# RViMLab/MICCAI2021_Cataract_semantic_segmentation

Measured on AMD Instinct MI355X. Metric: train frames/sec @540x960 OCRNet-HRNetw48, higher is better.
Workload: dtype f32 (convolutions with K >= 2048 and >= 192 output columns, and the 3x3 trunk convolutions of the HRNet widths: forward / backward-data of those with > 192 output columns: operands scaled by a per-tensor power of two and split into 2 fp16 planes (22 significant bits), 3 fp16 MFMA products; forward /

## Files before the change

include/catseg_debug.h:

```cpp
#ifndef CATSEG_DEBUG_H
#define CATSEG_DEBUG_H

#include "catseg.h"

#ifdef __cplusplus
extern "C" {
#endif

int catseg_debug_set_tile(int mi, int ni);
int catseg_debug_set_splits(int splits);
int catseg_debug_set_strided_multi(int on);
int catseg_debug_set_lovasz_prune(int on);
int catseg_debug_set_wgrad_direct(int on);

int catseg_debug_set_dconv3_blocks(int blocks);
int catseg_debug_set_dconv3_spec(int on);
int catseg_debug_set_dconv3_alt96(int on);
int catseg_debug_set_dwgrad3_blocks(int blocks);
int catseg_debug_set_dwgrad3_pl_blocks(int blocks);
int catseg_debug_set_dconv3_pl_slots(int slots);
int catseg_debug_set_dconv3_pl_pair(int mask);
int catseg_debug_dconv3_pl_occupancy(int C, int pair);
int catseg_debug_dwgrad3_pl_occupancy(int C);

int catseg_debug_set_h2w_slow_epilogue(int on);

int catseg_debug_set_b3_tile(int t);
int catseg_debug_plan_conv(const catseg_conv_desc* d, int op, int* out);

int catseg_debug_set_bilinear_bwd_fused(int on);
int catseg_debug_set_h2w_waves(int waves);

int catseg_debug_set_pconv1_wgrad_blocks(int n);

#ifdef __cplusplus
}
#endif
#endif
```

miccai2021_cataract_semantic_segmentation_amd/_lib.py:

```python
import ctypes as C
import os

import torch

_HERE = os.path.dirname(os.path.abspath(__file__))
LIB_PATH = os.environ.get("CATSEG_LIB") or os.path.join(_HERE, "libcatseg_hip.so")

if not os.path.exists(LIB_PATH):
    raise ImportError(
        "libcatseg_hip.so is missing (%s). Build it with `python -c 'import __graft_entry__ as g; g.build()'` "
        "or `make -C miccai2021_cataract_semantic_segmentation_amd/csrc`. There is no CPU fallback." % LIB_PATH)

lib = C.CDLL(LIB_PATH)

P, I, L, F, SZ = C.c_void_p, C.c_int, C.c_longlong, C.c_float, C.c_size_t


class ConvDesc(C.Structure):
    _fields_ = [(n, I) for n in ("B", "H", "W", "Cin", "Ho", "Wo", "Cout", "kh", "kw", "stride", "pad", "dil",
                                 "ldx", "ldy", "stem4", "groups")]


_SIGS = {
    "catseg_last_error": (C.c_char_p, []),
    "catseg_version": (I, []),
    "catseg_conv2d_fwd": (I, [P, P, P, P, P, I, P]),
    "catseg_conv2d_fwd_bnstats": (I, [P, P, P, P, P, I, P, SZ, P, P, P]),
    "catseg_conv2d_fwd_bf16x3_bnstats": (I, [P, P, P, P, P, I, P, SZ, P, P, P]),
    "catseg_bn_finalize": (I, [P, I, L, L, I, P, F, F, P, P, P, P, P]),
    "catseg_bn_finalize_counts": (I, [P, I, P, L, I, P, F, F, P, P, P, P, P]),
    "catseg_dconv3_supported": (I, [I]),
    "catseg_dconv3_wimg_bytes": (SZ, [I]),
    "catseg_dconv3_tiles": (I, [I, I, I, I, P, P]),
    "catseg_dconv3_prep": (I, [P, I, I, P, P]),
    "catseg_dconv3_layout": (I, [I, P, P]),
    "catseg_dwgrad3_supported": (I, [I]),
    "catseg_dwgrad3_workspace": (SZ, [I, I, I, I]),
    "catseg_dwgrad3": (I, [I, I, I, I, P, I, P, I, P, P, SZ, P]),
    "catseg_debug_set_dwgrad3_blocks": (I, [I]),
    "catseg_dconv3_prep_batch": (I, [P, I, P, P, P]),
    "catseg_dconv3": (I, [I, I, I, I, P, I, P, P, P, I, I, P, SZ, P, P]),
    "catseg_dconv3_bnbwd": (I, [I, I, I, I, P, I, P, P, I, P, I, P, P, P, P, SZ, P]),
    "catseg_dwgrad3_f16x2": (I, [I, I, I, I, P, I, P, P, I, P, P, P, SZ, P]),
    "catseg_dconv3_f16x2_wimg_bytes": (SZ, [I]),
    "catseg_dconv3_f16x2_prep_batch": (I, [P, I, P, P, P, P]),
    "catseg_dconv3_f16x2": (I, [I, I, I, I, P, I, P, P, P, P, P, I, I, P, SZ, P, P]),
    "catseg_dconv3_bnbwd_f16x2": (I, [I, I, I, I, P, I, P, P, P, P, I, P, I, P, P, P, P, SZ, P]),
    "catseg_dconv3_pl_supported": (I, [I]),
    "catseg_dconv3_pl_rows": (I, [I, I, I, I]),
    "catseg_planes_bytes": (SZ, [L, I]),
    "catseg_planes_from_f32": (I, [P, I, L, I, P, P, I, P]),
    "catseg_dconv3_pl": (I, [I, I, I, I, P, P, P, P, P, P, I, I, P, SZ, P, P, P]),
    "catseg_dconv3_pl_bnbwd": (I, [I, I, I, I, P, P, P, P, P, I, P, I, P, P, P, P, SZ, P, P]),
    "catseg_dwgrad3_pl_supported": (I, [I]),
    "catseg_dwgrad3_pl_workspace": (SZ, [I, I, I, I]),
    "catseg_dwgrad3_pl": (I, [I, I, I, I, P, P, P, P, P, P, SZ, P]),
    "catseg_bn_finalize_counts_bound": (I, [P, I, P, L, I, P, P, F, F, P, P, P, P, P, P, P]),
    "catseg_bn_apply_planes": (I, [P, I, P, P, P, P, I, P, P, I, P, L, I, I, P, P]),
    "catseg_add_n_act_planes": (I, [P, P, P, I, P, I, P, L, I, I, P, P]),
    "catseg_bn_backward_planes": (I, [P, I, P, I, P, I, P, P, P, L, I, I, P, P, P, P, P, P, P, I, I, P, SZ, P]),
    "catseg_bn_backward_pre_planes": (I, [P, I, P, I, P, P, P, I, L, I, P, P, P, P, P, P, P, SZ, P]),
    "catseg_bn_backward_h2_workspace": (SZ, [L, I]),
    "catseg_bn_backward_h2": (I, [P, I, P, I, P, I, P, P, P, L, I, I, P, P, P, P, P, P, P, P, P, SZ, P]),
    "catseg_head_fwd": (I, [P, I, P, P, P, P, P, I, L, I, P, I, I, P]),
    "catseg_head_backward_workspace": (SZ, [L, I]),
    "catseg_head_backward": (I, [P, I, P, I, P, P, P, P, I, L, I, P, P, P, P, P, P, P, P, P, P, P, SZ, P]),
    "catseg_head_fwd_drop": (I, [P, I, P, P, P, P, P, I, L, I, P, I, I, P, L, F, P]),
    "catseg_head_backward_drop": (I, [P, I, P, I, P, P, P, P, I, L, I, P, P, P, P, P, P, P, P, P, P, P, SZ, P, L, F, P]),
    "catseg_dropout2d_mask": (I, [P, F, I, I, P, P, P]),
    "catseg_dropout2d_mask_fixed": (I, [P, F, I, I, P, P, P]),
    "catseg_dropout2d_apply": (I, [P, I, P, L, I, L, P, I, P]),
    "catseg_maxpool2x2_fwd": (I, [P, I, P, I, P, I, I, I, I, P]),
    "catseg_maxpool2x2_bwd": (I, [P, I, P, P, I, I, I, I, I, P]),
    "catseg_bias_rows": (I, [P, P, I, L, I, P]),
    "catseg_bn_apply_amax": (I, [P, I, P, P, P, P, I, P, I, L, I, I, P, P]),
    "catseg_bn_backward_amax": (I, [P, I, P, I, P, I, P, P, P, L, I, I, P, I, P, P, P, I, I, P, SZ, P, P]),
    "catseg_bn_mask_bytes": (SZ, [L, I]),
    "catseg_bn_apply_mask": (I, [P, I, P, P, P, P, I, P, I, L, I, P, P, P]),
    "catseg_bn_backward_mask": (I, [P, I, P, P, I, P, P, L, I, P, I, P, P, P, I, I, P, SZ, P, P]),
    "catseg_bn_apply_planes_mask": (I, [P, I, P, P, P, P, I, P, P, I, P, L, I, P, P, P]),
    "catseg_bn_backward_planes_mask": (I, [P, I, P, P, I, P, P, L, I, P, P, P, P, P, P, P, I, I, P, SZ, P]),
    "catseg_bn_backward_pre_amax": (I, [P, I, P, I, P, P, P, I, L, I, P, I, P, P, P, SZ, P, P]),
    "catseg_add_n_act_amax": (I, [P, P, I, P, I, L, I, I, P, P]),
    "catseg_conv2d_fwd_fused": (I, [P, P, P, P, P, I, I, P, P]),
    "catseg_fold_bn": (I, [P, P, P, P, P, P, F, I, I, P, P, P]),
    "catseg_conv2d_bwd_data": (I, [P, P, P, P, I, P]),
    "catseg_conv2d_bwd_weight_workspace": (SZ, [P]),
    "catseg_conv2d_bwd_weight": (I, [P, P, P, P, P, P, SZ, P]),
    "catseg_gemm_batched": (I, [I, I, I, I, I, P, I, L, P, I, L, P, I, L, I, I, P]),
    "catseg_sum_slabs": (I, [P, P, L, I, I, I, P]),
    "catseg_debug_set_tile": (I, [I, I]),
    "catseg_debug_set_splits": (I, [I]),
    "catseg_debug_set_strided_multi": (I, [I]),
    "catseg_debug_set_lovasz_prune": (I, [I]),
    "catseg_debug_set_wgrad_direct": (I, [I]),
    "catseg_debug_plan_conv": (I, [P, I, P]),
    "catseg_debug_set_b3_tile": (I, [I]),
    "catseg_debug_set_dconv3_blocks": (I, [I]),
    "catseg_debug_set_dconv3_pl_slots": (I, [I]),
    "catseg_debug_set_dconv3_pl_pair": (I, [I]),
    "catseg_debug_set_dwgrad3_pl_blocks": (I, [I]),
    "catseg_debug_dconv3_pl_occupancy": (I, [I, I]),
    "catseg_debug_dwgrad3_pl_occupancy": (I, [I]),
    "catseg_debug_set_dconv3_spec": (I, [I]),
    "catseg_debug_set_dconv3_alt96": (I, [I]),
    "catseg_aug_pad_flip_u8": (I, [P, P, I, I, I, I, P, I, I, P]),
    "catseg_aug_box_blur": (I, [P, P, I, I, I, I, P, P, P, P]),
    "catseg_aug_color_op": (I, [P, I, I, I, P, P, P, SZ, P]),
    "catseg_split3_elems": (SZ, [L, I]),
    "catseg_split3": (I, [P, I, L, I, P, P]),
    "catseg_split3_weight_t": (I, [P, I, I, I, P, P]),
    "catseg_split3_blocked_elems": (SZ, [L, I]),
    "catseg_split3_blocked": (I, [P, L, I, I, P, P, P]),
    "catseg_split3_weight_blocked": (I, [P, I, I, I, P, P]),
    "catseg_split3_weight_t_blocked": (I, [P, I, I, I, P, P]),
    "catseg_conv2d_fwd_bf16x3_blocked": (I, [P, P, P, P, P, I, P, SZ, P, P, P]),
    "catseg_conv2d_bwd_data_bf16x3_blocked": (I, [P, P, P, P, I, P]),
    "catseg_conv2d_fwd_fused_bf16x3_blocked": (I, [P, P, P, P, P, I, I, P, P]),
    "catseg_split2h_blocked_elems": (SZ, [L, I]),
    "catseg_split2h_planar_elems": (SZ, [L, I]),
    "catseg_split2h": (I, [P, L, I, I, P, P, P, P]),
    "catseg_split2h_bound": (I, [P, L, I, I, P, P, P, P, P, P, P, P]),
    "catseg_conv2d_bwd_weight_f16x2_workspace": (SZ, [P]),
    "catseg_conv2d_bwd_weight_f16x2": (I, [P, P, P, P, P, P, P, SZ, P]),
    "catseg_conv2d_bwd_weight_f16x2_blocked": (I, [P, P, P, P, P, P, P, SZ, P]),
    "catseg_concat_bilinear_split2h": (I, [I, P, P, P, P, P, P, I, I, I, P, P, P]),
    "catseg_stem3_supported": (I, [I, I, I]),
    "catseg_stem3_partial_rows": (I, [I, I, I]),
    "catseg_stem3_wgrad_workspace": (SZ, []),
    "catseg_stem3_fwd": (I, [P, L, L, L, L, I, I, I, P, P, P, I, P, P, P]),
    "catseg_stem3_bwd_weight": (I, [P, L, L, L, L, I, I, I, P, I, P, P, SZ, P]),
    "catseg_stem7_supported": (I, [I, I, I]),
    "catseg_stem7_partial_rows": (I, [I, I, I]),
    "catseg_stem7_fwd": (I, [P, L, L, L, L, I, I, I, P, P, P, I, P, P, P]),
    "catseg_split2h_weight_blocked": (I, [P, I, I, I, P, P, P]),
    "catseg_split2h_weight_t_blocked": (I, [P, I, I, I, P, P, P]),
    "catseg_conv2d_fwd_f16x2_blocked": (I, [P, P, P, P, P, P, P, I, P, SZ, P, P, P]),
    "catseg_conv2d_fwd_fused_f16x2_blocked": (I, [P, P, P, P, P, P, P, I, I, P, P]),
    "catseg_conv2d_bwd_data_f16x2_blocked": (I, [P, P, P, P, P, P, I, P]),
    "catseg_conv2d_fwd_bf16x3": (I, [P, P, P, P, P, I, P]),
    "catseg_conv2d_bwd_data_bf16x3": (I, [P, P, P, P, I, P]),
    "catseg_conv2d_bwd_weight_bf16x3_workspace": (SZ, [P]),
    "catseg_conv2d_bwd_weight_bf16x3": (I, [P, P, P, P, P, SZ, P]),
    "catseg_bias_grad": (I, [P, I, L, I, P, P, SZ, P]),
    "catseg_bn_workspace": (SZ, [L, I]),
    "catseg_bn_train_stats": (I, [P, L, I, I, P, F, F, P, P, P, P, P, SZ, P]),
    "catseg_bn_eval_scale": (I, [I, P, P, F, P, P]),
    "catseg_bn_apply": (I, [P, I, P, P, P, P, I, P, I, L, I, I, P]),
    "catseg_bn_backward": (I, [P, I, P, I, P, I, P, P, P, L, I, I, P, I, P, P, P, I, I, P, SZ, P]),
    "catseg_bn_backward_pre": (I, [P, I, P, I, P, P, P, I, L, I, P, I, P, P, P, SZ, P]),
    "catseg_nchw3_to_nhwc4": (I, [P, P, I, I, I, P]),
    "catseg_nchw3_to_nhwc4_norm": (I, [P, P, I, I, I, P, P, P]),
    "catseg_stem_pack_weight": (I, [P, P, I, P]),
    "catseg_stem_unpack_grad": (I, [P, P, I, P]),
    "catseg_axpy2d": (I, [P, I, P, I, L, I, F, I, P]),
    "catseg_add_n_act": (I, [P, P, I, P, I, L, I, I, P]),
    "catseg_relu_bwd": (I, [P, I, P, I, P, I, L, I, P]),
    "catseg_weight_pad_cin": (I, [P, P, I, I, I, I, I, P]),
    "catseg_scale_by_device_scalar": (I, [P, L, P, P]),
    "catseg_maxpool3x3s2_fwd": (I, [P, I, P, I, P, I, I, I, I, I, I, P]),
    "catseg_maxpool3x3s2_bwd": (I, [P, I, P, P, I, I, I, I, I, I, I, P]),
    "catseg_bilinear_fwd": (I, [P, I, P, I, I, I, I, I, I, I, I, I, P]),
    "catseg_bilinear_bwd": (I, [P, I, P, I, I, I, I, I, I, I, I, I, I, P, SZ, P]),
    "catseg_global_avgpool_fwd": (I, [P, I, P, I, I, I, P]),
    "catseg_global_avgpool_bwd": (I, [P, P, I, I, I, I, I, P]),
    "catseg_adaptive_avgpool_fwd": (I, [P, I, P, I, I, I, I, I, P]),
    "catseg_adaptive_avgpool_bwd": (I, [P, P, I, I, I, I, I, I, I, P]),
    "catseg_softmax_spatial_workspace": (SZ, [I, I]),
    "catseg_softmax_spatial_fwd": (I, [P, P, I, I, I, I, P, SZ, P]),
    "catseg_softmax_spatial_bwd": (I, [P, P, P, I, I, I, I, I, P, SZ, P]),
    "catseg_softmax_rows_fwd": (I, [P, P, L, I, I, F, P]),
    "catseg_softmax_rows_bwd": (I, [P, P, P, L, I, I, F, P]),
    "catseg_lovasz_workspace": (SZ, [L, I]),
    "catseg_lovasz_softmax": (I, [P, P, L, I, F, P, P, I, P, SZ, P]),
    "catseg_lovasz_softmax_fwd": (I, [P, P, L, I, F, P, I, P, SZ, P]),
    "catseg_lovasz_softmax_bwd": (I, [P, L, I, F, P, P, I, P, SZ, P]),
    "catseg_ce_workspace": (SZ, [L]),
    "catseg_cross_entropy": (I, [P, P, L, I, L, F, P, P, P, SZ, P]),
    "catseg_ohem_workspace": (SZ, [L]),
    "catseg_ohem_cross_entropy": (I, [P, P, L, I, L, F, L, F, P, P, P, SZ, P]),
    "catseg_overlap_workspace": (SZ, [L, I]),
    "catseg_overlap_fwd": (I, [P, P, L, I, L, I, I, I, P, P, P, P, P, SZ, P]),
    "catseg_overlap_bwd": (I, [P, P, L, I, L, P, P, P, P]),
    "catseg_focal_workspace": (SZ, [L]),
    "catseg_focal_fwd": (I, [P, P, L, I, F, P, P, P, P, SZ, P]),
    "catseg_focal_bwd": (I, [P, P, L, I, F, P, P, P, P]),
    "catseg_ingest_u8": (I, [P, P, I, I, I, P, P, I, I, P, P, P, P, P, P]),
    "catseg_resize_nearest": (I, [P, I, P, I, I, I, I, I, I, I, I, I, F, P]),
    "catseg_ensemble_merge": (I, [P, P, I, L, I, I, P, I, P, P]),
    "catseg_confusion_matrix": (I, [P, P, L, I, P, P]),
    "catseg_adam_step": (I, [P, P, P, P, L, F, F, F, F, I, F, P]),
    "catseg_pconv1_supported": (I, [I, I]),
    "catseg_pconv1_wimg_bytes": (SZ, [I, I]),
    "catseg_pconv1_prep_batch": (I, [P, I, P, P, P, P]),
    "catseg_pconv1": (I, [L, I, I, P, I, P, P, P, P, P, I, I, P, SZ, P, P, P]),
    "catseg_pconv1_wgrad_supported": (I, [I, I]),
    "catseg_pconv1_wgrad_workspace": (SZ, [L, I, I]),
    "catseg_pconv1_wgrad": (I, [L, I, I, P, I, P, P, I, P, P, P, SZ, P]),
    "catseg_debug_set_pconv1_wgrad_blocks": (I, [I]),
    "catseg_debug_set_h2w_waves": (I, [I]),
    "catseg_debug_set_h2w_slow_epilogue": (I, [I]),
    "catseg_debug_set_bilinear_bwd_fused": (I, [I]),
    "catseg_gconv_supported": (I, [P]),
    "catseg_gconv_class_bytes": (SZ, [P]),
    "catseg_gconv_wimg_bytes": (SZ, [P, I]),
    "catseg_gconv_entries": (I, [P, I, L, L, P]),
    "catseg_gconv_fwd": (I, [P, P, P, P, P, P, P, P, SZ, P, P, P]),
    "catseg_gconv_bwd_data": (I, [P, P, P, P, P, P, I, P]),
    "catseg_gconv_wgrad_supported": (I, [P]),
    "catseg_gconv_wgrad_workspace": (SZ, [P]),
    "catseg_gconv_bwd_weight": (I, [P, P, P, P, P, P, P, SZ, P]),
    "catseg_adam_hyper": (None, [F, F, F, I, F, P]),
    "catseg_adam_step_dev": (I, [P, P, P, P, L, P, F, F, F, P]),
    "catseg_lds_limits": (I, [P, P]),
}
for _name, (_res, _args) in _SIGS.items():
    _fn = getattr(lib, _name)
    _fn.restype = _res
    _fn.argtypes = _args

EXPORTS = tuple(_SIGS)

if os.environ.get("CATSEG_SYNC"):
    class _SyncLib:
        def __init__(self, inner):
            self._inner = inner

        def __getattr__(self, name):
            fn = getattr(self._inner, name)
            if name in ("catseg_last_error", "catseg_version") or name.endswith("_workspace"):
                return fn

            def call(*a):
                desc = [[getattr(x._obj, f) for f, _ in x._obj._fields_] for x in a if isinstance(getattr(x, "_obj", None), ConvDesc)]
                print("[catseg]", name, desc, [x for x in a if isinstance(x, (int, float))], flush=True)
                rc = fn(*a)
                torch.cuda.synchronize()
                return rc
            return call

    lib = _SyncLib(lib)


class CatsegError(RuntimeError):
    pass


def check(rc):
    if rc != 0:
        raise CatsegError("libcatseg_hip: error %d: %s" % (rc, lib.catseg_last_error().decode()))


def stream():
    return torch.cuda.current_stream().cuda_stream


def ptr(t):
    return 0 if t is None else t.data_ptr()
```

miccai2021_cataract_semantic_segmentation_amd/csrc/dwgrad3_pl.hip:

```cpp
#include "planes.h"
#include "slabs.h"

extern int catseg_g_wg_blocks;
int catseg_g_wp96_blocks = 512;
extern "C" int catseg_debug_set_dwgrad3_pl_blocks(int blocks) {
  catseg_g_wp96_blocks = blocks > 0 ? blocks : 512;
  return CATSEG_OK;
}

namespace {

typedef _Float16 h8 __attribute__((ext_vector_type(8)));
typedef short s16x4 __attribute__((ext_vector_type(4)));
typedef short s16x8 __attribute__((ext_vector_type(8)));
typedef __attribute__((address_space(3))) s16x4 lds_s16x4;

constexpr int wp_rowbytes(int c) { return ((c * 2 / 32) & 1) ? c * 2 : c * 2 + 32; }

template <int COT_, int NCI_, int NTY_, int WM_, int WN_, int TH_, int NBUF_>
struct WpCfg {
  static constexpr int NBUF = NBUF_;
  static constexpr int COT = COT_, NCI = NCI_, NTY = NTY_, WM = WM_, WN = WN_, TH = TH_, TW = 16;
  static constexpr int NW = WM * WN, NTHR = 64 * NW;
  static_assert(NW == 4 && (TH == 2 || TH == 4), "four waves; tiles of 2 or 4 rows");
  static constexpr int MT = COT / 16 / WM;
  static constexpr int NTL = NTY * 3 * (NCI / 16);
  static constexpr int NTW = (NTL + WN - 1) / WN;
  static constexpr int XH = TH + NTY - 1, XW = TW + 2;
  static constexpr int NPX_X = XH * XW, NPX_D = TH * TW;
  static constexpr int ROWB_X = wp_rowbytes(NCI), ROWB_D = wp_rowbytes(COT);
  static constexpr int SX = ROWB_X / 16, SD = ROWB_D / 16;
  static constexpr int XPS = (NPX_X * ROWB_X + 255) / 256 * 256, DPS = (NPX_D * ROWB_D + 255) / 256 * 256;
  static constexpr int D0 = 2 * XPS, BUF = 2 * (XPS + DPS);
  static constexpr int LDS = NBUF * BUF;
  static constexpr int NKS = TH * TW / 32;
  static constexpr int NJX = (NPX_X * SX + 63) / 64, NJD = (NPX_D * SD + 63) / 64;
  static constexpr int MX = (NJX + 3) / 4, MD = (NJD + 3) / 4;
  static_assert(COT % (16 * WM) == 0 && NCI % 16 == 0 && (NTY == 1 || NTY == 3) && LDS <= 80 * 1024, "tiling");
};

struct WpArgs {
  const unsigned char* xp;
  const unsigned char* dp;
  unsigned P16;
  const int* x_rec;
  const int* d_rec;
  int B, H, W, C;
  int tiles_y, tiles_x, splits;
  float* slabs;
  long long slab_stride;
};

template <class G>
__global__ __launch_bounds__(G::NTHR, 2) void dwgrad3_pl_kernel(const WpArgs a) {
  __shared__ __attribute__((aligned(256))) unsigned char smem[G::LDS];
  const int tid = threadIdx.x, lane = tid & 63;
  const int wave = __builtin_amdgcn_readfirstlane(tid >> 6);
  const int wm = wave / G::WN, wn = wave % G::WN;
  const int i16 = lane & 15, kg = lane >> 4;

  const int nco = a.C / G::COT, nci = a.C / G::NCI;
  const int nvar = nco * nci * (G::NTY == 3 ? 1 : 3);
  const int split = (int)(blockIdx.x >> 3) / nvar * 8 + (int)(blockIdx.x & 7);
  if (split >= a.splits) return;
  int v = (int)(blockIdx.x >> 3) % nvar;
  const int cot0 = (v % nco) * G::COT; v /= nco;
  const int ci0 = (v % nci) * G::NCI; v /= nci;
  const int ky0 = G::NTY == 3 ? 0 : v;
  const int NG = a.C / 8;

  const int ntile = a.B * a.tiles_y * a.tiles_x;
  const int t_begin = (int)((long long)split * ntile / a.splits), t_end = (int)((long long)(split + 1) * ntile / a.splits);
  const int ex_x = __builtin_amdgcn_readfirstlane(a.x_rec[CS_REC_EXP]);
  const int ex_d = __builtin_amdgcn_readfirstlane(a.d_rec[CS_REC_EXP]);
  const bool one_step = ex_x + ex_d >= -120 && ex_x + ex_d <= 120;
  const float sc_out = __builtin_ldexpf(1.f, one_step ? -(ex_x + ex_d) : 0);

  int x_rel[G::MX], x_r[G::MX], x_c[G::MX], d_rel[G::MD], d_r[G::MD], d_c[G::MD];
  unsigned x_go[G::MX], d_go[G::MD];
#pragma unroll
  for (int m = 0; m < G::MX; ++m) {
    const int s = (wave + 4 * m) * 64 + lane, px = s / G::SX, g = s - px * G::SX;
    const bool live = px < G::NPX_X && g < G::NCI / 8;
    x_r[m] = live ? px / G::XW + ky0 - 1 : -(1 << 20);
    x_c[m] = px % G::XW - 1;
    x_rel[m] = ((px / G::XW + ky0 - 1) * a.W + (px % G::XW - 1)) * 16;
    x_go[m] = (unsigned)g * a.P16;
  }
#pragma unroll
  for (int m = 0; m < G::MD; ++m) {
    const int s = (wave + 4 * m) * 64 + lane, px = s / G::SD, g = s - px * G::SD;
    const bool live = px < G::NPX_D && g < G::COT / 8;
    d_r[m] = live ? px / G::TW : -(1 << 20);
    d_c[m] = px % G::TW;
    d_rel[m] = ((px / G::TW) * a.W + px % G::TW) * 16;
    d_go[m] = (unsigned)g * a.P16;
  }
  const unsigned plane_bytes = (unsigned)NG * a.P16;
  const __amdgpu_buffer_rsrc_t rsx = __builtin_amdgcn_make_buffer_rsrc((void*)a.xp, (short)0, (int)(2u * plane_bytes), 0x00020000);
  const __amdgpu_buffer_rsrc_t rsd = __builtin_amdgcn_make_buffer_rsrc((void*)a.dp, (short)0, (int)(2u * plane_bytes), 0x00020000);
  auto dma = [&](int tile, int buf) {
    const int tx = tile % a.tiles_x, ty = (tile / a.tiles_x) % a.tiles_y, b = tile / (a.tiles_x * a.tiles_y);
    const int y0 = ty * G::TH, x0 = tx * G::TW;
    const int org = (y0 * a.W + x0) * 16;
    const unsigned img = (unsigned)(b * a.H * a.W) * 16u;
    unsigned char* base = smem + buf * G::BUF;
#pragma unroll
    for (int m = 0; m < G::MX; ++m) {
      const int j = wave + 4 * m;
      if (j < G::NJX) {
        const bool ok = (unsigned)(y0 + x_r[m]) < (unsigned)a.H && (unsigned)(x0 + x_c[m]) < (unsigned)a.W;
        const unsigned voff = ok ? (unsigned)(org + x_rel[m]) + x_go[m] : 0xFFFFFFF0u;
#pragma unroll
        for (int p = 0; p < 2; ++p)
          if (j * 64 + lane < G::NPX_X * G::SX)
            __builtin_amdgcn_raw_ptr_buffer_load_lds(rsx, (__attribute__((address_space(3))) void*)(base + p * G::XPS + j * 1024), 16, voff,
                                                     (unsigned)(p * NG + ci0 / 8) * a.P16 + img, 0, 0);
      }
    }
#pragma unroll
    for (int m = 0; m < G::MD; ++m) {
      const int j = wave + 4 * m;
      if (j < G::NJD) {
        const bool ok = (unsigned)(y0 + d_r[m]) < (unsigned)a.H && (unsigned)(x0 + d_c[m]) < (unsigned)a.W;
        const unsigned voff = ok ? (unsigned)(org + d_rel[m]) + d_go[m] : 0xFFFFFFF0u;
#pragma unroll
        for (int p = 0; p < 2; ++p)
          if (j * 64 + lane < G::NPX_D * G::SD)
            __builtin_amdgcn_raw_ptr_buffer_load_lds(rsd, (__attribute__((address_space(3))) void*)(base + G::D0 + p * G::DPS + j * 1024), 16, voff,
                                                     (unsigned)(p * NG + cot0 / 8) * a.P16 + img, 0, 0);
      }
    }
  };

  const int q = (lane >> 2) & 3, pp = lane & 3;
  const int a_base = G::D0 + (4 * kg + q) * G::ROWB_D + wm * G::MT * 32 + pp * 8;
  const int b_base = (4 * kg + q) * G::ROWB_X + pp * 8;
  int noff[G::NTW];
#pragma unroll
  for (int j = 0; j < G::NTW; ++j) {
    const int n = wn + j * G::WN;
    const int ct = n % (G::NCI / 16), kx = (n / (G::NCI / 16)) % 3, kyl = n / (3 * (G::NCI / 16));
    noff[j] = (kyl * G::XW + kx) * G::ROWB_X + ct * 32;
  }

  f32x4 acc[G::MT][G::NTW];
#pragma unroll
  for (int mt = 0; mt < G::MT; ++mt)
#pragma unroll
    for (int j = 0; j < G::NTW; ++j) acc[mt][j] = f32x4{0.f, 0.f, 0.f, 0.f};

  auto tread = [&](int addr) { return __builtin_amdgcn_ds_read_tr16_b64_v4i16((lds_s16x4*)(smem + addr)); };
  auto frag = [&](int addr, int hstride) {
    const s16x4 lo = tread(addr), hi = tread(addr + hstride);
    const s16x8 v8 = {lo[0], lo[1], lo[2], lo[3], hi[0], hi[1], hi[2], hi[3]};
    return __builtin_bit_cast(h8, v8);
  };

  int n_items = 0;
#pragma unroll
  for (int m = 0; m < G::MX; ++m) n_items += (wave + 4 * m < G::NJX) ? 2 : 0;
#pragma unroll
  for (int m = 0; m < G::MD; ++m) n_items += (wave + 4 * m < G::NJD) ? 2 : 0;
  auto wait_vm = [&](int n) {
    switch (n) {
      case 0: __builtin_amdgcn_s_waitcnt(0x0F70); break;
      case 2: __builtin_amdgcn_s_waitcnt(0x0F72); break;
      case 4: __builtin_amdgcn_s_waitcnt(0x0F74); break;
      case 6: __builtin_amdgcn_s_waitcnt(0x0F76); break;
      case 8: __builtin_amdgcn_s_waitcnt(0x0F78); break;
      case 10: __builtin_amdgcn_s_waitcnt(0x0F7A); break;
      case 12: __builtin_amdgcn_s_waitcnt(0x0F7C); break;
      default: __builtin_amdgcn_s_waitcnt(0x0F70); break;
    }
  };
#pragma unroll
  for (int i = 0; i < G::NBUF - 1; ++i)
    if (t_begin + i < t_end) dma(t_begin + i, i);
  if (t_begin + G::NBUF - 2 < t_end) wait_vm((G::NBUF - 2) * n_items);
  else __builtin_amdgcn_s_waitcnt(0x0F70);
  __syncthreads();
  int buf = 0, nbuf = G::NBUF - 1;
#pragma unroll 1
  for (int tile = t_begin; tile < t_end; ++tile) {
    if (tile + G::NBUF - 1 < t_end) dma(tile + G::NBUF - 1, nbuf);
    const int bo = buf * G::BUF;
#pragma unroll
    for (int ks = 0; ks < G::NKS; ++ks) {
      h8 af[G::MT][2];
#pragma unroll
      for (int mt = 0; mt < G::MT; ++mt)
#pragma unroll
        for (int p = 0; p < 2; ++p) af[mt][p] = frag(bo + a_base + ks * 32 * G::ROWB_D + mt * 32 + p * G::DPS, 16 * G::ROWB_D);
#pragma unroll
      for (int j = 0; j < G::NTW; ++j) {
        if (wn + j * G::WN < G::NTL) {
          h8 bf[2];
#pragma unroll
          for (int p = 0; p < 2; ++p) bf[p] = frag(bo + b_base + ks * 2 * G::XW * G::ROWB_X + noff[j] + p * G::XPS, G::XW * G::ROWB_X);
#pragma unroll
          for (int mt = 0; mt < G::MT; ++mt) {
            f32x4 c = acc[mt][j];
            c = __builtin_amdgcn_mfma_f32_16x16x32_f16(af[mt][0], bf[1], c, 0, 0, 0);
            c = __builtin_amdgcn_mfma_f32_16x16x32_f16(af[mt][1], bf[0], c, 0, 0, 0);
            c = __builtin_amdgcn_mfma_f32_16x16x32_f16(af[mt][0], bf[0], c, 0, 0, 0);
            acc[mt][j] = c;
          }
        }
      }
    }
    if (tile + G::NBUF - 1 < t_end) wait_vm((G::NBUF - 2) * n_items);
    else __builtin_amdgcn_s_waitcnt(0x0F70);
    __syncthreads();
    buf = buf + 1 == G::NBUF ? 0 : buf + 1;
    nbuf = nbuf + 1 == G::NBUF ? 0 : nbuf + 1;
  }

  float* out = a.slabs + (long long)split * a.slab_stride;
#pragma unroll
  for (int mt = 0; mt < G::MT; ++mt)
#pragma unroll
    for (int j = 0; j < G::NTW; ++j) {
      const int n = wn + j * G::WN;
      if (n < G::NTL) {
        const int ct = n % (G::NCI / 16), kx = (n / (G::NCI / 16)) % 3, ky = ky0 + n / (3 * (G::NCI / 16));
#pragma unroll
        for (int r = 0; r < 4; ++r) {
          const int o = cot0 + (wm * G::MT + mt) * 16 + 4 * kg + r;
          out[((long long)(o * 3 + ky) * 3 + kx) * a.C + ci0 + ct * 16 + i16] =
              one_step ? acc[mt][j][r] * sc_out : __builtin_ldexpf(__builtin_ldexpf(acc[mt][j][r], -ex_x), -ex_d);
        }
      }
    }
}

using Wp48 = WpCfg<48, 48, 3, 1, 4, 4, 2>;
using Wp96 = WpCfg<96, 48, 1, 2, 2, 2, 2>;

struct WpPlan { int kind, variants, splits, TH; };

WpPlan wp_plan(int C, int B, int H, int W) {
  WpPlan p = {0, 0, 0, 0};
  if (C == 48) { p.kind = 1; p.variants = 1; p.TH = Wp48::TH; }
  else if (C == 96 || C == 192 || C == 384) { p.kind = 2; p.variants = (C / Wp96::COT) * (C / Wp96::NCI) * (Wp96::NTY == 3 ? 1 : 3); p.TH = Wp96::TH; }
  else return p;
  const int ntile = B * ((H + p.TH - 1) / p.TH) * ((W + 15) / 16);
  int s = (p.kind == 2 ? catseg_g_wp96_blocks : catseg_g_wg_blocks) / p.variants;
  if (s < 1) s = 1;
  if (s > ntile) s = ntile;
  p.splits = s;
  return p;
}

}

extern "C" int catseg_dwgrad3_pl_supported(int C) { return C == 48 || C == 96 || C == 192 || C == 384; }

extern "C" int catseg_debug_dwgrad3_pl_occupancy(int C) {
  int n = -1;
  hipError_t e = C == 48 ? hipOccupancyMaxActiveBlocksPerMultiprocessor(&n, dwgrad3_pl_kernel<Wp48>, Wp48::NTHR, 0)
                         : hipOccupancyMaxActiveBlocksPerMultiprocessor(&n, dwgrad3_pl_kernel<Wp96>, Wp96::NTHR, 0);
  return e == hipSuccess ? n : -1;
}

extern "C" size_t catseg_dwgrad3_pl_workspace(int B, int H, int W, int C) {
  const WpPlan p = wp_plan(C, B, H, W);
  return p.kind ? (size_t)p.splits * C * 9 * C * 4 : 0;
}

extern "C" int catseg_dwgrad3_pl(int B, int H, int W, int C, const void* x_planes, const void* x_record, const void* dy_planes,
                                 const void* dy_record, float* dw, void* workspace, size_t workspace_bytes, catseg_stream_t stream) {
  const WpPlan p = wp_plan(C, B, H, W);
  CS_REQUIRE(p.kind, "dwgrad3 (planes): unsupported channel count %d", C);
  CS_REQUIRE(B > 0 && H > 0 && W > 0 && x_planes && dy_planes && x_record && dy_record && dw && workspace, "dwgrad3 (planes): bad args");
  CS_REQUIRE(cs_aligned16(x_planes) && cs_aligned16(dy_planes) && cs_aligned16(dw) && cs_aligned16(workspace), "dwgrad3 (planes): alignment");
  const long long P = (long long)B * H * W;
  CS_REQUIRE(4 * P * C < (1LL << 32), "dwgrad3 (planes): tensor too large for 32-bit offsets");
  const long long wel = (long long)C * 9 * C;
  if (workspace_bytes < (size_t)p.splits * wel * 4) {
    catseg_set_error("dwgrad3 (planes): workspace %zu < %zu", workspace_bytes, (size_t)p.splits * wel * 4);
    return CATSEG_EWORKSPACE;
  }
  WpArgs a;
  a.xp = (const unsigned char*)x_planes; a.dp = (const unsigned char*)dy_planes; a.P16 = (unsigned)(P * 16);
  a.x_rec = (const int*)x_record; a.d_rec = (const int*)dy_record;
  a.B = B; a.H = H; a.W = W; a.C = C;
  a.tiles_y = (H + p.TH - 1) / p.TH;
  a.tiles_x = (W + 15) / 16;
  a.slabs = (float*)workspace;
  a.slab_stride = wel;
  a.splits = p.splits;
  hipStream_t st = (hipStream_t)stream;
  const int grid = (p.splits + 7) / 8 * 8 * p.variants;
  if (p.kind == 1) hipLaunchKernelGGL((dwgrad3_pl_kernel<Wp48>), dim3(grid), dim3(Wp48::NTHR), 0, st, a);
  else hipLaunchKernelGGL((dwgrad3_pl_kernel<Wp96>), dim3(grid), dim3(Wp96::NTHR), 0, st, a);
  const long long n4 = wel / 4;
  cs_launch_reduce_slabs4((const float*)workspace, dw, n4, p.splits, st);
  CS_LAUNCH_CHECK();
  return CATSEG_OK;
}
```

Before: 81.74.

## Add alternative 3x3 weight-gradient tilings and inline-asm LDS DMA; default to 48x48 full-ky

Adds several alternative tile configurations for the planes-based 3x3 weight-gradient kernel at 96/192/384 channels, selectable through a new debug form switch. The default now uses a 48-output by 48-input tile that covers all three kernel rows in one block, instead of 96x48 with one kernel row per block. It also adds an inline-assembly buffer-load-to-LDS path that sets M0 by hand. The intent is better reuse of the loaded activation and gradient tiles and fewer variant blocks. The risk is that split counts are still derived from the old variant count, which changes the grid size, and the hand-written M0 handling may add scheduling overhead.

```diff
diff --git a/include/catseg_debug.h b/include/catseg_debug.h
--- a/include/catseg_debug.h
+++ b/include/catseg_debug.h
@@ -18,6 +18,7 @@
 int catseg_debug_set_dconv3_alt96(int on);
 int catseg_debug_set_dwgrad3_blocks(int blocks);
 int catseg_debug_set_dwgrad3_pl_blocks(int blocks);
+int catseg_debug_set_dwgrad3_pl_form(int form);
 int catseg_debug_set_dconv3_pl_slots(int slots);
 int catseg_debug_set_dconv3_pl_pair(int mask);
 int catseg_debug_dconv3_pl_occupancy(int C, int pair);
diff --git a/miccai2021_cataract_semantic_segmentation_amd/_lib.py b/miccai2021_cataract_semantic_segmentation_amd/_lib.py
--- a/miccai2021_cataract_semantic_segmentation_amd/_lib.py
+++ b/miccai2021_cataract_semantic_segmentation_amd/_lib.py
@@ -100,6 +100,7 @@
     "catseg_debug_set_dconv3_pl_slots": (I, [I]),
     "catseg_debug_set_dconv3_pl_pair": (I, [I]),
     "catseg_debug_set_dwgrad3_pl_blocks": (I, [I]),
+    "catseg_debug_set_dwgrad3_pl_form": (I, [I]),
     "catseg_debug_dconv3_pl_occupancy": (I, [I, I]),
     "catseg_debug_dwgrad3_pl_occupancy": (I, [I]),
     "catseg_debug_set_dconv3_spec": (I, [I]),
diff --git a/miccai2021_cataract_semantic_segmentation_amd/csrc/dwgrad3_pl.hip b/miccai2021_cataract_semantic_segmentation_amd/csrc/dwgrad3_pl.hip
--- a/miccai2021_cataract_semantic_segmentation_amd/csrc/dwgrad3_pl.hip
+++ b/miccai2021_cataract_semantic_segmentation_amd/csrc/dwgrad3_pl.hip
@@ -7,6 +7,12 @@
   catseg_g_wp96_blocks = blocks > 0 ? blocks : 512;
   return CATSEG_OK;
 }
+constexpr int WP96_FORM = 3;
+int catseg_g_wp96_form = WP96_FORM;
+extern "C" int catseg_debug_set_dwgrad3_pl_form(int form) {
+  catseg_g_wp96_form = form >= 0 && form <= 4 ? form : WP96_FORM;
+  return CATSEG_OK;
+}
 
 namespace {
 
@@ -17,8 +23,17 @@
 
 constexpr int wp_rowbytes(int c) { return ((c * 2 / 32) & 1) ? c * 2 : c * 2 + 32; }
 
-template <int COT_, int NCI_, int NTY_, int WM_, int WN_, int TH_, int NBUF_>
+typedef int i32x4 __attribute__((ext_vector_type(4)));
+
+__device__ __forceinline__ void wp_dma16(i32x4 rsrc, unsigned lds, unsigned voff, unsigned soff) {
+  unsigned keep;
+  asm volatile("s_mov_b32 %0, m0\n\ts_mov_b32 m0, %1\n\ts_nop 0\n\tbuffer_load_dwordx4 %2, %3, %4 offen lds\n\ts_mov_b32 m0, %0"
+               : "=&s"(keep) : "s"(lds), "v"(voff), "s"(rsrc), "s"(soff) : "memory");
+}
+
+template <int COT_, int NCI_, int NTY_, int WM_, int WN_, int TH_, int NBUF_, bool LATE_ = false>
 struct WpCfg {
+  static constexpr bool LATE = LATE_;
   static constexpr int NBUF = NBUF_;
   static constexpr int COT = COT_, NCI = NCI_, NTY = NTY_, WM = WM_, WN = WN_, TH = TH_, TW = 16;
   static constexpr int NW = WM * WN, NTHR = 64 * NW;
@@ -99,6 +114,12 @@
   const unsigned plane_bytes = (unsigned)NG * a.P16;
   const __amdgpu_buffer_rsrc_t rsx = __builtin_amdgcn_make_buffer_rsrc((void*)a.xp, (short)0, (int)(2u * plane_bytes), 0x00020000);
   const __amdgpu_buffer_rsrc_t rsd = __builtin_amdgcn_make_buffer_rsrc((void*)a.dp, (short)0, (int)(2u * plane_bytes), 0x00020000);
+  auto raw_rsrc = [&](const unsigned char* ptr) {
+    const unsigned long long v = (unsigned long long)ptr;
+    return i32x4{(int)(unsigned)v, (int)((unsigned)(v >> 32) & 0xFFFFu), (int)(2u * plane_bytes), 0x00020000};
+  };
+  const i32x4 rax = raw_rsrc(a.xp), rad = raw_rsrc(a.dp);
+  auto lds_addr = [&](unsigned char* ptr) { return (unsigned)(unsigned long long)(__attribute__((address_space(3))) unsigned char*)ptr; };
   auto dma = [&](int tile, int buf) {
     const int tx = tile % a.tiles_x, ty = (tile / a.tiles_x) % a.tiles_y, b = tile / (a.tiles_x * a.tiles_y);
     const int y0 = ty * G::TH, x0 = tx * G::TW;
@@ -113,9 +134,12 @@
         const unsigned voff = ok ? (unsigned)(org + x_rel[m]) + x_go[m] : 0xFFFFFFF0u;
 #pragma unroll
         for (int p = 0; p < 2; ++p)
-          if (j * 64 + lane < G::NPX_X * G::SX)
+          if (j * 64 + lane < G::NPX_X * G::SX) {
+            if constexpr (G::LATE) wp_dma16(rax, lds_addr(base + p * G::XPS + j * 1024), voff, (unsigned)(p * NG + ci0 / 8) * a.P16 + img);
+            else
             __builtin_amdgcn_raw_ptr_buffer_load_lds(rsx, (__attribute__((address_space(3))) void*)(base + p * G::XPS + j * 1024), 16, voff,
                                                      (unsigned)(p * NG + ci0 / 8) * a.P16 + img, 0, 0);
+          }
       }
     }
 #pragma unroll
@@ -126,9 +150,12 @@
         const unsigned voff = ok ? (unsigned)(org + d_rel[m]) + d_go[m] : 0xFFFFFFF0u;
 #pragma unroll
         for (int p = 0; p < 2; ++p)
-          if (j * 64 + lane < G::NPX_D * G::SD)
+          if (j * 64 + lane < G::NPX_D * G::SD) {
+            if constexpr (G::LATE) wp_dma16(rad, lds_addr(base + G::D0 + p * G::DPS + j * 1024), voff, (unsigned)(p * NG + cot0 / 8) * a.P16 + img);
+            else
             __builtin_amdgcn_raw_ptr_buffer_load_lds(rsd, (__attribute__((address_space(3))) void*)(base + G::D0 + p * G::DPS + j * 1024), 16, voff,
                                                      (unsigned)(p * NG + cot0 / 8) * a.P16 + img, 0, 0);
+          }
       }
     }
   };
@@ -236,20 +263,35 @@
 
 using Wp48 = WpCfg<48, 48, 3, 1, 4, 4, 2>;
 using Wp96 = WpCfg<96, 48, 1, 2, 2, 2, 2>;
+using Wp96L = WpCfg<96, 48, 1, 2, 2, 2, 2, true>;
+using Wp96R = WpCfg<96, 48, 3, 2, 2, 2, 2, true>;
+using Wp48R = WpCfg<48, 48, 3, 1, 4, 2, 2, true>;
+using Wp96RB = WpCfg<96, 48, 3, 2, 2, 2, 2>;
 
 struct WpPlan { int kind, variants, splits, TH; };
+
+template <class G> constexpr int wp_variants(int C) { return (C / G::COT) * (C / G::NCI) * (G::NTY == 3 ? 1 : 3); }
 
 WpPlan wp_plan(int C, int B, int H, int W) {
   WpPlan p = {0, 0, 0, 0};
   if (C == 48) { p.kind = 1; p.variants = 1; p.TH = Wp48::TH; }
-  else if (C == 96 || C == 192 || C == 384) { p.kind = 2; p.variants = (C / Wp96::COT) * (C / Wp96::NCI) * (Wp96::NTY == 3 ? 1 : 3); p.TH = Wp96::TH; }
+  else if (C == 96 || C == 192 || C == 384) { p.kind = 2; p.variants = wp_variants<Wp96>(C); p.TH = Wp96::TH; }
   else return p;
   const int ntile = B * ((H + p.TH - 1) / p.TH) * ((W + 15) / 16);
   int s = (p.kind == 2 ? catseg_g_wp96_blocks : catseg_g_wg_blocks) / p.variants;
   if (s < 1) s = 1;
   if (s > ntile) s = ntile;
   p.splits = s;
+  if (p.kind == 2) {
+    p.kind += catseg_g_wp96_form;
+    p.variants = p.kind == 4 || p.kind == 6 ? wp_variants<Wp96R>(C) : p.kind == 5 ? wp_variants<Wp48R>(C) : p.variants;
+  }
   return p;
+}
+
+template <class G> hipError_t wp_occupancy(int* n) { return hipOccupancyMaxActiveBlocksPerMultiprocessor(n, dwgrad3_pl_kernel<G>, G::NTHR, 0); }
+template <class G> void wp_launch(int grid, hipStream_t st, const WpArgs& a) {
+  hipLaunchKernelGGL((dwgrad3_pl_kernel<G>), dim3(grid), dim3(G::NTHR), 0, st, a);
 }
 
 }
@@ -258,8 +300,9 @@
 
 extern "C" int catseg_debug_dwgrad3_pl_occupancy(int C) {
   int n = -1;
-  hipError_t e = C == 48 ? hipOccupancyMaxActiveBlocksPerMultiprocessor(&n, dwgrad3_pl_kernel<Wp48>, Wp48::NTHR, 0)
-                         : hipOccupancyMaxActiveBlocksPerMultiprocessor(&n, dwgrad3_pl_kernel<Wp96>, Wp96::NTHR, 0);
+  const int form = C == 48 ? -1 : catseg_g_wp96_form;
+  hipError_t e = form < 0 ? wp_occupancy<Wp48>(&n) : form == 0 ? wp_occupancy<Wp96>(&n) : form == 1 ? wp_occupancy<Wp96L>(&n)
+                 : form == 2 ? wp_occupancy<Wp96R>(&n) : form == 3 ? wp_occupancy<Wp48R>(&n) : wp_occupancy<Wp96RB>(&n);
   return e == hipSuccess ? n : -1;
 }
 
@@ -292,8 +335,14 @@
   a.splits = p.splits;
   hipStream_t st = (hipStream_t)stream;
   const int grid = (p.splits + 7) / 8 * 8 * p.variants;
-  if (p.kind == 1) hipLaunchKernelGGL((dwgrad3_pl_kernel<Wp48>), dim3(grid), dim3(Wp48::NTHR), 0, st, a);
-  else hipLaunchKernelGGL((dwgrad3_pl_kernel<Wp96>), dim3(grid), dim3(Wp96::NTHR), 0, st, a);
+  switch (p.kind) {
+    case 1: wp_launch<Wp48>(grid, st, a); break;
+    case 2: wp_launch<Wp96>(grid, st, a); break;
+    case 3: wp_launch<Wp96L>(grid, st, a); break;
+    case 4: wp_launch<Wp96R>(grid, st, a); break;
+    case 5: wp_launch<Wp48R>(grid, st, a); break;
+    default: wp_launch<Wp96RB>(grid, st, a); break;
+  }
   const long long n4 = wel / 4;
   cs_launch_reduce_slabs4((const float*)workspace, dw, n4, p.splits, st);
   CS_LAUNCH_CHECK();
```

After: 82.68 (median of 6 runs). +1.2%, better.
